# zyc00/Point-SAM

Hardware: AMD Instinct MI355X
Metric: point-clouds/sec (encode+1-prompt decode) (higher is better)
Workload: dtype f32 (fp32 in/out/accumulate; large GEMMs as row-scaled 2-way fp16 split x 3 MFMA products, fp32-grade error)

## Files before the change

### include/pointsam_hip.h

```cpp
#ifndef POINTSAM_HIP_H
#define POINTSAM_HIP_H

#include <stddef.h>
#include <stdint.h>

#ifdef __cplusplus
extern "C" {
#endif

typedef struct ihipStream_t* psam_stream_t;

#define PSAM_OK 0
#define PSAM_EINVAL (-1)
#define PSAM_EALIGN (-2)
#define PSAM_EWORKSPACE (-3)

#define PSAM_ACT_NONE 0
#define PSAM_ACT_GELU 1
#define PSAM_ACT_RELU 2
#define PSAM_ACT_SWIGLU 3

int32_t psam_version(void);
const char* psam_last_error_string(void);

// ... 62 lines not shown
#endif
#define PSAM_COUNTER_BYTES 65536
void psam_attention_f16x3_force_keysplit(int32_t mode);
int32_t psam_attention_f16x3_last_instance(void);
int32_t psam_attention_f16x3_last_keysplit(void);
int32_t psam_attention_f32_last_instance(void);
#ifdef PSAM_BUILD_EXPERIMENTS
void psam_twoway_decoder_force_fork(int32_t mode);
#endif
int32_t psam_gemm_f16x3p_fused_row_ln(int32_t N);
typedef struct {
    float* out_scale; float out_k1, out_k2; int32_t pack_out;
    float* stats; int32_t stat_cols;
    const float* ln_mean; const float* ln_rstd; const float* ln_c;
    float* gmax_out; int64_t gmax_ld; int32_t gmax_k; int32_t no_store;
    const float* row_ln_g; const float* row_ln_b; float row_ln_eps;
    const float* hyper; float* masks; int32_t hyper_c; int32_t hyper_rows;
    int64_t hyper_pstride;
    float* splitk_ws; int64_t splitk_plane; int32_t splitk;
    const float* out_bound;
    int32_t* counters;
} psam_gemm_fuse_t;
int32_t psam_gemm_f16x3p_splitk(int32_t M, int32_t N, int32_t K, int32_t act);
int32_t psam_gemm_f16x3p_hyper_planes(int32_t N, int32_t with_row_ln);
int32_t psam_sum_planes(const float* parts, int32_t P, int64_t pstride, int64_t count, float* out, psam_stream_t stream);
int32_t psam_gemm_f16x3p_stat_segs(int32_t N);
int32_t psam_gemm_f16x3p_ex(const void* A, int64_t lda, const float* scaleA, const void* W, int64_t ldw, const float* scaleW, float* C, int64_t ldc,
                            const float* bias, const float* residual, int64_t ldr, const float* rowbias, int64_t ldrb, int32_t rowgroup, int32_t M,
                            int32_t N, int32_t K, float alpha, int32_t act, const psam_gemm_fuse_t* fuse, psam_stream_t stream);
int32_t psam_ln_stats_finalize(const float* stats, int32_t rows, int32_t segs, int32_t cols, float eps, float* mean, float* rstd, psam_stream_t stream);
int32_t psam_linear128_ln_gelu_pack(const void* x, int64_t ldx, const float* x_scale, const void* w, int64_t ldw, const float* w_scale, const float* rowbias,
                                    int64_t ldrb, int32_t rowgroup, const float* gamma, const float* beta, float eps, float bound, int64_t rows, int32_t h1,
                                    void* out, int64_t ldo, float* out_scale, psam_stream_t stream);
int32_t psam_scale_pack_rows_g8(const float* X, int64_t ldx, int32_t rows, int32_t K, void* P, int64_t ldp, float* scale, psam_stream_t stream);
int32_t psam_linear(const float* x, int64_t ldx, const float* W, int64_t ldw, const float* bias, const float* residual, int64_t ldr, float* y,
                    int64_t ldy, int32_t M, int32_t N, int32_t K, int32_t act, psam_stream_t stream);
void psam_gemm_bf16x6_force_config(int32_t cfg);
void psam_gemm_force_config(int32_t cfg);

int32_t psam_layernorm(const float* x, int64_t ldx, const float* res, int64_t ldr, const float* w, const float* b, float* y, int64_t ldy,
                       int64_t rows, int32_t cols, float eps, int32_t act, psam_stream_t stream);
int32_t psam_layernorm_ex(const float* x, int64_t ldx, const float* res, int64_t ldr, const float* w, const float* b, float* y, int64_t ldy,
                          int64_t rows, int32_t cols, float eps, int32_t act, float* row_scale, int32_t pack, psam_stream_t stream);
int32_t psam_layernorm_ex2(const float* x, int64_t ldx, const float* res, int64_t ldr, const float* w, const float* b, float* y, int64_t ldy,
                           int64_t rows, int32_t cols, float eps, int32_t act, float* row_scale, int32_t pack, float* row_bound, float c2,
                           float c1, float c0, psam_stream_t stream);
int32_t psam_layernorm_rs(const float* x, int64_t ldx, const float* res, int64_t ldr, const float* w, const float* b, float* y, int64_t ldy,
                          int64_t rows, int32_t cols, float eps, int32_t act, float* row_scale, psam_stream_t stream);
int32_t psam_layernorm_last_instance(void);

int32_t psam_swiglu_ln(const float* gx, int64_t ldg, int32_t xoff, const float* w, const float* b, float* out, int64_t ldo, int64_t rows,
                       int32_t H, float eps, psam_stream_t stream);
int32_t psam_swiglu_ln_last_instance(void);

int32_t psam_attention_f32(const float* q, int64_t ldq, int64_t sq, const float* k, int64_t ldk, int64_t sk, const float* v, int64_t ldv,
                           int64_t sv, float* o, int64_t ldo, int64_t so, int32_t B, int32_t H, int32_t Lq, int32_t Lk, int32_t hd,
                           float scale, psam_stream_t stream);
int32_t psam_attention_f16x3(const float* q, int64_t ldq, int64_t sq, const float* k, int64_t ldk, int64_t sk, const float* v, int64_t ldv,
                           int64_t sv, float* o, int64_t ldo, int64_t so, int32_t B, int32_t H, int32_t Lq, int32_t Lk, int32_t hd,
                           float scale, psam_stream_t stream);
int32_t psam_attention_f16x3_ex(const float* q, int64_t ldq, int64_t sq, const float* k, int64_t ldk, int64_t sk, const float* v, int64_t ldv,
                                int64_t sv, float* o, int64_t ldo, int64_t so, int32_t B, int32_t H, int32_t Lq, int32_t Lk, int32_t hd, float scale,
                                const float* a_scale, float k1, float k2, float* o_scale, psam_stream_t stream);
size_t psam_attention_f16x3_keysplit_ws_bytes(int32_t B, int32_t H, int32_t Lq, int32_t Lk, int32_t hd, int32_t max_keysplit);
int32_t psam_attention_f16x3_ex2(const float* q, int64_t ldq, int64_t sq, const float* k, int64_t ldk, int64_t sk, const float* v, int64_t ldv,
                                int64_t sv, float* o, int64_t ldo, int64_t so, int32_t B, int32_t H, int32_t Lq, int32_t Lk, int32_t hd, float scale,
// ... 291 lines not shown
```

### point_sam_amd/_lib.py

```python
import ctypes
import os

_HERE = os.path.dirname(os.path.abspath(__file__))
LIB_PATH = os.environ.get("PSAM_HIP_LIB") or os.path.join(_HERE, "csrc", "libpointsam_hip.so")

i32, i64, f32 = ctypes.c_int32, ctypes.c_int64, ctypes.c_float
ptr, size_t = ctypes.c_void_p, ctypes.c_size_t

SIGNATURES = {
    "psam_version": (i32, []),
    "psam_last_error_string": (ctypes.c_char_p, []),
    "psam_fps_workspace_bytes": (size_t, [i32, i32, i32]),
    "psam_fps_set_cooperative": (None, [i32]),
    "psam_fps_set_pruning": (None, [i32]),
    "psam_fps": (i32, [ptr, i32, i32, i32, ptr, ptr, ptr, size_t, ptr]),
    "psam_knn": (i32, [ptr, ptr, i32, i32, i32, i32, ptr, ptr]),
    "psam_fps_last_instance": (i32, []),
    "psam_fps_last_grid_x": (i32, []),
    "psam_knn_force_band": (None, [i32]),
    "psam_knn_last_instance": (i32, []),
    "psam_three_nn": (i32, [ptr, ptr, i32, i32, i32, f32, ptr, ptr, ptr]),
    "psam_group_gather": (i32, [ptr, ptr, ptr, ptr, i32, i32, i32, i32, i32, i32, ptr, ptr]),
    "psam_group_gather_r": (i32, [ptr, ptr, ptr, ptr, i32, i32, i32, i32, i32, i32, f32, ptr, ptr]),
    "psam_group_gather_ld": (i32, [ptr, ptr, ptr, ptr, i32, i32, i32, i32, i32, i32, f32, ptr, i64, ptr]),
    "psam_patch_l1": (i32, [ptr, ptr, ptr, ptr, ptr, ptr, ptr, ptr, f32, i32, i32, i32, i32, i32, i32, ptr, ptr]),
    "psam_patch_l1_r": (i32, [ptr, ptr, ptr, ptr, ptr, ptr, ptr, ptr, f32, i32, i32, i32, i32, i32, i32, f32, ptr, ptr]),
    "psam_patch_l1_ex": (i32, [ptr, ptr, ptr, ptr, ptr, ptr, ptr, ptr, ptr, f32, i32, i32, i32, i32, i32, i32, f32, ptr, ptr, ptr]),
    "psam_error_regions": (i32, [ptr, ptr, ptr, ptr, i64, ptr]),
    "psam_border_farthest_workspace_bytes": (size_t, [i32, i32]),
    "psam_border_farthest": (i32, [ptr, ptr, i32, i32, i32, ptr, ptr, ptr, size_t, ptr]),
    "psam_group_max": (i32, [ptr, i64, ptr, i64, i64, i32, i32, ptr]),
    "psam_gemm_f32": (i32, [ptr, i64, i64, i64, ptr, i64, i64, i64, ptr, i64, i64, i64, ptr, ptr, i64, i64, i64, ptr, i64, i32,
                            i32, i32, i32, i32, i32, f32, i32, ptr]),
    "psam_gemm_bf16x6": (i32, [ptr, i64, i64, i64, ptr, i64, i64, i64, ptr, i64, i64, i64, ptr, ptr, i64, i64, i64, ptr, i64, i32,
                               i32, i32, i32, i32, i32, f32, i32, ptr]),
    "psam_linear": (i32, [ptr, i64, ptr, i64, ptr, ptr, i64, ptr, i64, i32, i32, i32, i32, ptr]),
    "psam_gemm_force_config": (None, [i32]),
    "psam_gemm_bf16x6_force_config": (None, [i32]),
    "psam_row_scale_f16": (i32, [ptr, i64, i32, i32, ptr, ptr]),
    "psam_pack_rows_f16x2_g8": (i32, [ptr, i64, ptr, i32, i32, ptr, i64, ptr]),
    "psam_gemm_f16x3p": (i32, [ptr, i64, ptr, ptr, i64, ptr, ptr, i64, ptr, ptr, i64, ptr, i64, i32, i32, i32, i32, f32, i32, ptr]),
    "psam_gemm_f16x3p_force_config": (None, [i32]),
    "psam_gemm_f16x3p_last_config": (i32, []),
    "psam_gemm_f16x3p_last_splitk": (i32, []),
    "psam_gemm_f16x3p_force_epilogue": (None, [i32]),
    "psam_gemm_f16x3p_force_splitk_fixup": (None, [i32]),
    "psam_gemm_f16x3p_force_continuous": (None, [i32]),
    "psam_attention_f16x3_force_keysplit": (None, [i32]),
    "psam_attention_f16x3_last_instance": (i32, []),
    "psam_attention_f16x3_last_keysplit": (i32, []),
    "psam_attention_f32_last_instance": (i32, []),
    "psam_twoway_decoder_force_fork": (None, [i32]),
    "psam_attention_packed_force_variant": (None, [i32]),
    "psam_attention_packed_force_nw": (None, [i32]),
    "psam_attention_packed_last_instance": (i32, []),
    "psam_gemm_f16x3p_fused_row_ln": (i32, [i32]),
    "psam_linear128_ln_gelu_pack": (i32, [ptr, i64, ptr, ptr, i64, ptr, ptr, i64, i32, ptr, ptr, f32, f32, i64, i32, ptr, i64, ptr, ptr]),
    "psam_gemm_f16x3p_stat_segs": (i32, [i32]),
    "psam_gemm_f16x3p_splitk": (i32, [i32, i32, i32, i32]),
    "psam_nn_group_feats": (i32, [ptr, ptr, ptr, ptr, ptr, i32, i32, i32, i32, i32, i32, ptr, i64, ptr]),
    "psam_scatter_amax": (i32, [ptr, i64, ptr, i64, i32, i64, i64, i32, ptr, i64, i32, ptr]),
    "psam_eva_block_prepared_bytes": (size_t, [i32, i32]),
    "psam_eva_block_prepare": (i32, [ptr, ptr, ptr, size_t, ptr]),
    "psam_eva_block_ws_bytes": (size_t, [i64, i32, i32]),
    "psam_eva_block": (i32, [ptr, ptr, ptr, i32, i32, ptr, size_t, ptr]),
    "psam_linear_skinny_multi": (i32, [ptr, i64, i64, i64, i32, i32, ptr]),
    "psam_linear_skinny_ln": (i32, [ptr, i64, ptr, i64, ptr, ptr, i64, ptr, ptr, f32, ptr, ptr, i64, i32, i32, i32, ptr, ptr]),
    "psam_linear_rows_multi": (i32, [ptr, i64, i64, i32, i32, i64, i64, i32, ptr]),
    "psam_linear_ln256": (i32, [ptr, i64, ptr, i64, ptr, ptr, i64, ptr, ptr, f32, ptr, i64, i64, i32, i32, ptr]),
    "psam_twoway_decoder_force_fast": (None, [i32]),
    "psam_scale_pack_rows_g8_add_dual": (i32, [ptr, i64, ptr, i64, i32, i32, i32, i32, ptr, ptr, ptr, ptr, i64, ptr]),
    "psam_mlp3_pair": (i32, [ptr, ptr, i32, ptr]),
    "psam_attention_small_force_split": (None, [i32]),
    "psam_attention_small_last_instance": (i32, []),
    "psam_layernorm_last_instance": (i32, []),
    "psam_swiglu_ln_last_instance": (i32, []),
    "psam_patch_l1_last_instance": (i32, []),
    "psam_interp3_last_instance": (i32, []),
    "psam_linear_skinny_ln_tmp_floats": (ctypes.c_size_t, [i32, i32]),
    "psam_scale_pack_rows_g8_add": (i32, [ptr, i64, ptr, i64, i32, i32, i32, i32, ptr, i64, ptr, ptr]),
    "psam_eva_gelu_block_prepared_bytes": (size_t, [i32, i32]),
    "psam_eva_gelu_block_prepare": (i32, [ptr, ptr, ptr, size_t, ptr]),
    "psam_eva_gelu_block_ws_bytes": (size_t, [i64, i32, i32]),
    "psam_eva_gelu_block": (i32, [ptr, ptr, ptr, i32, i32, ptr, size_t, ptr, ptr]),
    "psam_patch_encoder_prepared_bytes": (size_t, [i32, i32, i32]),
    "psam_patch_encoder_prepare": (i32, [ptr, ptr, ptr, size_t, ptr]),
    "psam_patch_encoder_ws_bytes": (size_t, [i64, i64, i32, i32]),
    "psam_patch_encoder": (i32, [ptr, ptr, ptr, ptr, ptr, ptr, ptr, i32, i32, i32, i32, i32, i32, f32, ptr, ptr, size_t, ptr]),
    "psam_upscale_masks_prepared_bytes": (size_t, [i32]),
    "psam_upscale_masks_prepare": (i32, [ptr, ptr, ptr, size_t, ptr]),
# ... 211 lines not shown
```

### point_sam_amd/build.py

```python
import os
import subprocess
import sys
from concurrent.futures import ThreadPoolExecutor

CSRC = os.path.join(os.path.dirname(os.path.abspath(__file__)), "csrc")
LIB = os.path.join(CSRC, "libpointsam_hip.so")
HIPCC = os.environ.get("HIPCC", "/opt/rocm/bin/hipcc")
ARCH = "gfx950"
COMMON = ["--offload-arch=" + ARCH, "-O3", "-std=c++17", "-fPIC", "-fvisibility=hidden", "-Wall", "-Wno-unused-function"]
EXPERIMENTS = os.environ.get("PSAM_BUILD_EXPERIMENTS", "0") == "1"
SOURCES = [
    ("tokenizer.hip", ["-ffp-contract=off"]),
    ("gemm.hip", []),
    ("gemm_split.hip", []),
    ("gemm_f16x3p.hip", []),
    ("gemm_f16x3pp.hip", []),
    ("patch_rowln.hip", []),
    ("attention.hip", []),
    ("rowops.hip", []),
    ("blocks.hip", []),
    ("masks.hip", []),
    ("scene.hip", ["-ffp-contract=off"]),
    ("regions.hip", ["-ffp-contract=off"]),
    ("crops.hip", ["-ffp-contract=off"]),
    ("scene_interp.hip", ["-ffp-contract=off"]),
    ("transfer.hip", ["-ffp-contract=off", "-fno-slp-vectorize"]),
    ("align.hip", ["-ffp-contract=off", "-fno-slp-vectorize"]),
    ("views.hip", ["-ffp-contract=off", "-fno-slp-vectorize"]),
    ("frames.hip", ["-ffp-contract=off", "-fno-slp-vectorize"]),
    ("fusion.hip", ["-ffp-contract=off", "-fno-slp-vectorize"]),
    ("geometry.hip", ["-ffp-contract=off", "-fno-slp-vectorize"]),
    ("error.cpp", ["-x", "hip"]),
] + ([("experiments/gemm_f16x3q.hip", ["-I" + CSRC]), ("experiments/gemm_f16x3s.hip", ["-I" + CSRC]), ("experiments/gemm_f16x3c.hip", ["-I" + CSRC]),
        ("experiments/twoway.hip", ["-I" + CSRC])] if EXPERIMENTS else [])
if EXPERIMENTS:
    COMMON = COMMON + ["-DPSAM_BUILD_EXPERIMENTS"]
FLAGS_STAMP = os.path.join(CSRC, ".build_flags")
PROBE_SRC = os.path.join(CSRC, "probe", "mfma_probe.hip")
PROBE_LIB = os.path.join(CSRC, "probe", "libpsam_probe.so")


def _stale(out, deps):
    return not os.path.exists(out) or any(os.path.getmtime(d) > os.path.getmtime(out) for d in deps)


def build_library(force: bool = False, verbose: bool = False) -> str:
    hdrs = [os.path.join(CSRC, f) for f in sorted(os.listdir(CSRC)) if f.endswith(".h")]
    hdrs.append(os.path.join(os.path.dirname(os.path.dirname(CSRC)), "include", "pointsam_hip.h"))
    flags = " ".join(COMMON)
    if (open(FLAGS_STAMP).read() != flags) if os.path.exists(FLAGS_STAMP) else EXPERIMENTS:
# ... 41 lines not shown
```

### point_sam_amd/csrc/blocks.hip

```cpp
#include <algorithm>
#include <cmath>
#include <cstring>
#include <initializer_list>
#ifdef PSAM_BUILD_EXPERIMENTS
#include <map>
#include <mutex>
#endif
#include <string>
#include <utility>
#include <vector>
#include "g8_pack.h"

namespace {
constexpr int64_t align256(int64_t b) { return (b + 255) / 256 * 256; }

struct Carve {
    char* base; int64_t off = 0;
    explicit Carve(void* p) : base(static_cast<char*>(p)) {}
    template <typename T> T* take(int64_t count) { T* r = base ? reinterpret_cast<T*>(base + off) : nullptr; off += align256(count * (int64_t)sizeof(T)); return r; }
    int64_t offset_of(const void* p) const { return static_cast<const char*>(p) - base; }
};
template <typename F> size_t carved_bytes(F&& layout) { Carve cv(nullptr); layout(cv); return (size_t)cv.off; }

struct Packed { float* w; float* s; };
// ... 401 lines not shown
    put_offsets(cv, p.c13, &plan->o_w13, &plan->o_s13); put_offsets(cv, p.c20m, &plan->o_w20m, &plan->o_s20m);
    put_offsets(cv, p.c20x, &plan->o_w20x, &plan->o_s20x); put_offsets(cv, p.c23, &plan->o_w23, &plan->o_s23);
    int32_t rc = pack_weight(WHO, wt->c13_w, h0, h0, h0, p.c13, stream);
    if (!rc) rc = pack_weight(WHO, wt->c20_w, 2 * h0, h1, h0, p.c20m, stream);
    if (!rc) rc = pack_weight(WHO, wt->c20_w + h0, 2 * h0, h1, h0, p.c20x, stream);
    if (!rc) rc = pack_weight(WHO, wt->c23_w, h1, cout, h1, p.c23, stream);
    return packing_done(WHO, rc, stream);
#undef WHO
}

PSAM_API size_t psam_patch_encoder_ws_bytes(int64_t rows, int64_t groups, int32_t h0, int32_t h1) {
    if (rows <= 0 || groups <= 0 || h0 <= 0 || h1 <= 0) return 0;
    return carved_bytes([&](Carve& cv) { patch_ws(cv, rows, groups, h0, h1); });
}

PSAM_API int32_t psam_patch_encoder(const psam_patch_encoder_plan_t* plan, const void* prepared, const float* xyz, const float* feats, const float* centers,
                                    const int64_t* knn_idx, const int64_t* center_idx, int32_t B, int32_t rep, int32_t N, int32_t G, int32_t K, int32_t C,
                                    float radius, float* out, void* ws, size_t ws_bytes, hipStream_t stream) {
    PSAM_REQUIRE(plan && prepared && xyz && feats && centers && knn_idx && out && ws, PSAM_EINVAL, "psam_patch_encoder: null pointer");
    const int h0 = plan->h0, h1 = plan->h1, cout = plan->cout, a = kpad32(h0), b = kpad32(h1);
    const int64_t groups = (int64_t)B * rep * G, rows = groups * K;
    PSAM_REQUIRE(B > 0 && rep > 0 && N > 0 && G > 0 && (K == 32 || (K > 0 && K % 64 == 0)) && rows % 256 == 0 && rows < ((int64_t)1 << 31), PSAM_EINVAL,
                 "psam_patch_encoder: group size must be 32 or a multiple of 64, and B * rep * G * K a multiple of 256");
    const int Kp = K <= 64 ? K : 64, parts = K / Kp;
    PSAM_REQUIRE(plan->cin == 3 + C * (center_idx ? 2 : 1), PSAM_EINVAL, "psam_patch_encoder: feature channels do not match the first Linear");
    PSAM_REQUIRE(ws_bytes >= psam_patch_encoder_ws_bytes(rows, groups, h0, h1), PSAM_EWORKSPACE, "psam_patch_encoder: workspace too small");
    auto P = [&](int64_t off) { return at(prepared, off); };
    Carve cv(ws);
    const PatchWs w = patch_ws(cv, rows, groups, h0, h1);
    float* part1 = parts > 1 ? w.x3 : w.y1;
    float* part2 = parts > 1 ? w.x1 : out;
    PSAM_REQUIRE(parts == 1 || ((int64_t)groups * parts * h0 <= rows * b && (int64_t)groups * parts * cout <= rows * a), PSAM_EINVAL,
                 "psam_patch_encoder: partial maxima do not fit the workspace");
    int32_t rc = psam_patch_l1_ex(xyz, feats, centers, knn_idx, center_idx, plan->c10_w, plan->c10_b, plan->c11_w, plan->c11_b, plan->eps, B, rep, N, G, K, C, radius, w.x1, w.s1, stream);
    if (rc) return rc;
    psam_gemm_fuse_t f;
    std::memset(&f, 0, sizeof(f));
    f.pack_out = 1; f.out_scale = w.s2; f.out_k1 = plan->k1; f.out_k2 = plan->k2; f.gmax_out = part1; f.gmax_ld = h0; f.gmax_k = Kp;
    rc = psam_gemm_f16x3p_ex(w.x1, a, w.s1, P(plan->o_w13), a, P(plan->o_s13), w.x2, a, plan->c13_b, nullptr, 0, nullptr, 0, 0, (int32_t)rows, h0, a, 1.f, 0, &f, stream);
    if (rc) return rc;
    if (parts > 1) { rc = psam_group_max(part1, h0, w.y1, h0, groups, parts, h0, stream); if (rc) return rc; }
    const Lin c20m{plan->c20_w, 2 * h0, plan->c20_b, P(plan->o_w20m), P(plan->o_s20m), h1, h0};
    rc = host_linear(c20m, w.y1, groups, w.g1, 0, G, w.y1p, w.sy, stream);
    if (rc) return rc;
    if (h1 == 512 && rows % 128 == 0 && psam_gemm_f16x3p_fused_row_ln(h1)) {
        std::memset(&f, 0, sizeof(f));
        f.row_ln_g = plan->c21_w; f.row_ln_b = plan->c21_b; f.row_ln_eps = plan->eps; f.pack_out = 1; f.out_scale = w.rs; f.out_k1 = 0.f; f.out_k2 = plan->ln21_bound;
        rc = psam_gemm_f16x3p_ex(w.x2, a, w.s2, P(plan->o_w20x), a, P(plan->o_s20x), w.x3, b, nullptr, nullptr, 0, w.g1, h1, K, (int32_t)rows, h1, a, 1.f, PSAM_ACT_GELU, &f, stream);
        if (rc) return rc;
    } else if (h0 == 128 && h1 == 512 && rows % 64 == 0) {
        rc = psam_linear128_ln_gelu_pack(w.x2, a, w.s2, P(plan->o_w20x), a, P(plan->o_s20x), w.g1, h1, K, plan->c21_w, plan->c21_b, plan->eps, plan->ln21_bound, rows, h1,
                                         w.x3, b, w.rs, stream);
        if (rc) return rc;
    } else {
        rc = psam_gemm_f16x3p_ex(w.x2, a, w.s2, P(plan->o_w20x), a, P(plan->o_s20x), w.x3, h1, nullptr, nullptr, 0, w.g1, h1, K, (int32_t)rows, h1, a, 1.f, 0, nullptr, stream);
        if (rc) return rc;
        rc = psam_layernorm_ex(w.x3, h1, nullptr, 0, plan->c21_w, plan->c21_b, w.x3, b, rows, h1, plan->eps, PSAM_ACT_GELU, w.rs, 1, stream);
        if (rc) return rc;
    }
    std::memset(&f, 0, sizeof(f));
    f.gmax_out = part2; f.gmax_ld = cout; f.gmax_k = Kp; f.no_store = 1;
    rc = psam_gemm_f16x3p_ex(w.x3, b, w.rs, P(plan->o_w23), b, P(plan->o_s23), out, cout, plan->c23_b, nullptr, 0, nullptr, 0, 0, (int32_t)rows, cout, b, 1.f, 0, &f, stream);
    if (rc || parts == 1) return rc;
    return psam_group_max(part2, cout, out, cout, groups, parts, cout, stream);
}

namespace {
struct UpscalePrepared { Packed u0, u3; };
UpscalePrepared upscale_prepared(Carve& cv, int dim) { return {take_packed(cv, dim, dim), take_packed(cv, dim, dim)}; }

struct UpscaleWs { float *kp, *k1, *sk, *up, *s1, *parts; };
UpscaleWs upscale_ws(Carve& cv, int64_t Z, int N, int G, int C, int dim) {
    const int64_t a = kpad32(dim), planes = psam_gemm_f16x3p_hyper_planes(dim, 0);
// ... 416 lines not shown
```

### point_sam_amd/csrc/g8_pack.h

```cpp
#pragma once
#include "common.h"

typedef unsigned u32x4 __attribute__((ext_vector_type(4)));

static inline __host__ __device__ int kpad32(int k) { return (k + 31) & ~31; }

#ifdef __HIPCC__
typedef float psam_f32x2 __attribute__((ext_vector_type(2)));
typedef float psam_f32x4 __attribute__((ext_vector_type(4)));
typedef _Float16 psam_f16x2 __attribute__((ext_vector_type(2)));

__device__ __forceinline__ void g8_split2_scaled(const psam_f32x2 xs, unsigned& hi, unsigned& lo) {
    const psam_f16x2 h = __builtin_convertvector(xs, psam_f16x2);
    const psam_f32x2 r = xs - __builtin_convertvector(h, psam_f32x2);
    hi = __builtin_bit_cast(unsigned, h);
    lo = __builtin_bit_cast(unsigned, __builtin_convertvector(r, psam_f16x2));
}
__device__ __forceinline__ void psam_split2_f16(float x0, float x1, float s, unsigned& hi, unsigned& lo) { g8_split2_scaled(psam_f32x2{x0, x1} * s, hi, lo); }

__device__ __forceinline__ float g8_absmax4(const psam_f32x4 v) { return fmaxf(fmaxf(fabsf(v[0]), fabsf(v[1])), fmaxf(fabsf(v[2]), fabsf(v[3]))); }
__device__ __forceinline__ float g8_absmax4(float amax, const psam_f32x4 v) { return fmaxf(fmaxf(amax, fmaxf(fabsf(v[0]), fabsf(v[1]))), fmaxf(fabsf(v[2]), fabsf(v[3]))); }
__device__ __forceinline__ float g8_row_scale(float lane_max) { return f16_row_scale(wave_max(lane_max)); }

template <int DIST, bool SHFL = false>
// ... 26 lines not shown
    g8_split2_scaled(xs23, h1, l1);
    return g8_chunk_words<DIST>(h0, l0, h1, l1, lane);
}

struct g8_group { u32x4 hi, lo; };
__device__ __forceinline__ g8_group g8_halfwave_group(const psam_f32x4 x, const psam_f32x4 y, float s) {
    unsigned xh[2], xl[2], yh[2], yl[2];
    psam_split2_f16(x[0], x[1], s, xh[0], xl[0]);
    psam_split2_f16(x[2], x[3], s, xh[1], xl[1]);
    psam_split2_f16(y[0], y[1], s, yh[0], yl[0]);
    psam_split2_f16(y[2], y[3], s, yh[1], yl[1]);
    psam_swap32(xh[0], yh[0]); psam_swap32(xh[1], yh[1]); psam_swap32(xl[0], yl[0]); psam_swap32(xl[1], yl[1]);
    return {u32x4{xh[0], xh[1], yh[0], yh[1]}, u32x4{xl[0], xl[1], yl[0], yl[1]}};
}
__device__ __forceinline__ g8_group g8_whole_group(const float (&v)[8], float s) {
    unsigned hi[4], lo[4];
#pragma unroll
    for (int e = 0; e < 4; ++e) psam_split2_f16(v[2 * e], v[2 * e + 1], s, hi[e], lo[e]);
    return {u32x4{hi[0], hi[1], hi[2], hi[3]}, u32x4{lo[0], lo[1], lo[2], lo[3]}};
}
__device__ __forceinline__ void g8_store_group(unsigned* first, const g8_group& g) {
    *reinterpret_cast<u32x4*>(first) = g.hi;
    *reinterpret_cast<u32x4*>(first + 4) = g.lo;
}
__device__ __forceinline__ void g8_store_halfwave_group(unsigned* first, const psam_f32x4 x, const psam_f32x4 y, float s) { g8_store_group(first, g8_halfwave_group(x, y, s)); }

__device__ __forceinline__ void g8_store_pair(unsigned* P, int64_t row, int ld, int lane, float x0, float x1, float s) {
    unsigned hi, lo;
    psam_split2_f16(x0, x1, s, hi, lo);
    unsigned* o = P + row * ld + (lane >> 2) * 8 + (lane & 3);
    o[0] = hi;
    o[4] = lo;
}
#endif
```

### point_sam_amd/model.py

```python
import math
from dataclasses import dataclass, field
from types import SimpleNamespace
from typing import Optional

import torch

from . import ops
from .config import ModelConfig
from .ops import ACT_GELU, ACT_NONE, ACT_RELU
from .streams import pipeline_streams
from .weights import check_state_dict


def _round_up(x, m):
    return (x + m - 1) // m * m


@dataclass
class TokenizerState:
    fps_idx: torch.Tensor
    centers: torch.Tensor
    knn_idx: torch.Tensor
    interp_index: torch.Tensor
    interp_weight: torch.Tensor
# ... 162 lines not shown
            if cfg.vit.swiglu and ops.EvaBlock.supported(D, cfg.vit.heads, cfg.vit.mlp_hidden):
                for blk in self.blocks:
                    blk.c_block = ops.EvaBlock(w, blk.p, D, cfg.vit.heads, cfg.vit.mlp_hidden, cfg.vit.ln_eps)
            elif not cfg.vit.swiglu and ops.EvaGeluBlock.supported(D, cfg.vit.heads, cfg.vit.mlp_hidden):
                for blk in self.blocks:
                    blk.c_block = ops.EvaGeluBlock(w, blk.p, D, cfg.vit.heads, cfg.vit.mlp_hidden, cfg.vit.ln_eps)
            torch.cuda.current_stream(self.device).synchronize()

    def _lin(self, name, x, **kw):
        return ops.linear(x, self.fw.get(name + ".weight", self.w[name + ".weight"]), self.w.get(name + ".bias"), **kw)

    def _ln(self, name, x, eps, **kw):
        return ops.layernorm(x, self.w[name + ".weight"], self.w[name + ".bias"], eps, **kw)

    def _ln_feeds_gemm(self, x, consumer):
        if self.precision != "f16x3" or x.shape[0] < ops.SPLIT_MIN_M or (consumer + ".weight") not in self.fw or not ops.layernorm_can_pack(x.shape[1]) \
                or x.shape[1] % 32 != 0:
            return False, None
        return True, torch.empty(x.shape[0], dtype=torch.float32, device=x.device)

    def _patch_encoder(self, prefix, coords, feats, centers, knn_idx, radius=None, center_idx=None):
        w, eps = self.w, self.cfg.ln_eps
        K = knn_idx.shape[2]
        h0 = self.cfg.patch_hidden[0]
        rows = feats.shape[0] * knn_idx.shape[1] * K
        l1 = (w[prefix + ".conv1.0.weight"], w[prefix + ".conv1.0.bias"], w[prefix + ".conv1.1.weight"], w[prefix + ".conv1.1.bias"], eps)
        w2a = w[prefix + ".conv2.0.weight"]
        fused = (self.precision == "f16x3" and self.fuse_patch and (K in (32, 64) or K % 64 == 0) and ops.fuse_supported(rows, 128) and prefix in self.pe_bound
                 and all((prefix + n) in self.fw for n in (".conv1.3.weight", ".conv2.0.weight#x", ".conv2.3.weight")))
        if fused and self.c_blocks and prefix in getattr(self, "c_patch", {}) and ops.current_gemm_mode() == "f16x3":
            return self.c_patch[prefix].run(coords, feats, centers, knn_idx, radius=radius, center_idx=center_idx)
        if fused:
            groups = rows // K
            s1 = torch.empty(rows, dtype=torch.float32, device=coords.device)
            h1 = ops.patch_l1(coords, feats, centers, knn_idx, *l1, radius=radius, center_idx=center_idx, scale_out=s1)
            h2 = torch.empty(rows, h0, dtype=torch.float32, device=coords.device)
            s2 = torch.empty(rows, dtype=torch.float32, device=coords.device)
            Kp = K if K <= 64 else 64
            parts = K // Kp
            y1 = torch.empty(groups * parts, h0, dtype=torch.float32, device=coords.device)
            k1, k2 = self.pe_bound[prefix]
            self._lin(prefix + ".conv1.3", h1, x_scale=s1, x_packed=True, out=h2, pack_out=(s2, k1, k2), group_max_out=y1, group_max_k=Kp)
            if parts > 1:
                y1 = ops.group_max(y1, parts)
            del h1
            g1 = ops.linear(y1, self.fw.get(prefix + ".conv2.0.weight#max", w2a[:, :h0]), w[prefix + ".conv2.0.bias"])
            hd1 = w2a.shape[0]
            if ops.fused_row_ln(hd1) and hd1 == 512 and (prefix + ".conv2.3.weight") in self.fw and rows % 128 == 0:
                h3 = torch.empty(rows, hd1, dtype=torch.float32, device=coords.device)
                rs, pk = torch.empty(rows, dtype=torch.float32, device=coords.device), True
                bound = self.ln_bound.get(prefix)
                if bound is None:
                    bound = self.ln_bound.setdefault(prefix, 1.001 * ops.row_ln_bound(w[prefix + ".conv2.1.weight"], w[prefix + ".conv2.1.bias"]) + 1e-30)
                ops.linear(h2, self.fw[prefix + ".conv2.0.weight#x"], None, act=ACT_GELU, rowbias=g1, rowgroup=K, x_scale=s2, x_packed=True, out=h3,
                           row_ln=(w[prefix + ".conv2.1.weight"], w[prefix + ".conv2.1.bias"], eps), pack_out=(rs, 0.0, bound))
                del h2
            elif ops.linear128_ln_gelu_supported(rows, h0, hd1, K) and (prefix + ".conv2.3.weight") in self.fw and ops.current_gemm_mode() == "f16x3":
                h3 = torch.empty(rows, hd1, dtype=torch.float32, device=coords.device)
                rs, pk = torch.empty(rows, dtype=torch.float32, device=coords.device), True
                bound = self.ln_bound.get(prefix)
                if bound is None:
                    bound = self.ln_bound.setdefault(prefix, 1.001 * ops.row_ln_bound(w[prefix + ".conv2.1.weight"], w[prefix + ".conv2.1.bias"]) + 1e-30)
                ops.linear128_ln_gelu_pack(h2, s2, self.fw[prefix + ".conv2.0.weight#x"], g1, K, w[prefix + ".conv2.1.weight"], w[prefix + ".conv2.1.bias"], eps, bound,
                                           h3, rs)
                del h2
            else:
                h3 = ops.linear(h2, self.fw[prefix + ".conv2.0.weight#x"], None, rowbias=g1, rowgroup=K, x_scale=s2, x_packed=True)
                del h2
                pk, rs = self._ln_feeds_gemm(h3, prefix + ".conv2.3")
                self._ln(prefix + ".conv2.1", h3, eps, act=ACT_GELU, out=h3, scale_out=rs, pack=pk)
            emb = torch.empty(groups * parts, self.w[prefix + ".conv2.3.weight"].shape[0], dtype=torch.float32, device=coords.device)
            self._lin(prefix + ".conv2.3", h3, x_scale=rs, x_packed=pk, group_max_out=emb, group_max_k=Kp, no_store=True)
            return ops.group_max(emb, parts) if parts > 1 else emb
        h1 = ops.patch_l1(coords, feats, centers, knn_idx, *l1, radius=radius, center_idx=center_idx)
        h2 = self._lin(prefix + ".conv1.3", h1)
        del h1
        y1 = ops.group_max(h2, K)
        g1 = ops.linear(y1, self.fw.get(prefix + ".conv2.0.weight#max", w2a[:, :h0]), w[prefix + ".conv2.0.bias"])
# ... 539 lines not shown
```

### point_sam_amd/ops.py

```python
import ctypes
import torch

from . import _lib
from ._lib import check

ACT_NONE, ACT_GELU, ACT_RELU, ACT_SWIGLU = 0, 1, 2, 3

GEMM_PROFILE = None
GEMM_PROFILE_EVERY = 29
GEMM_PROFILE_OTHERS = ()
GEMM_PROFILE_AFTER = 0
_gemm_counter = 0


def _sample_now():
    return GEMM_PROFILE is not None and _gemm_counter > GEMM_PROFILE_AFTER and _gemm_counter % GEMM_PROFILE_EVERY == 0


def _sampled_launch(launch, record):
    cur = torch.cuda.current_stream()
    for o in GEMM_PROFILE_OTHERS:
        cur.wait_stream(o)
    s, e = torch.cuda.Event(enable_timing=True), torch.cuda.Event(enable_timing=True)
    s.record()
# ... 168 lines not shown
    check(_lib.load().psam_three_nn(xyz.data_ptr(), centers.data_ptr(), B, N, G, eps, idx.data_ptr(), w.data_ptr(), _stream()), "psam_three_nn")
    return idx, w


def group_gather(xyz, feats, centers, knn_idx, radius=None, width=None):
    _chk(xyz); _chk(feats); _chk(centers); _chk(knn_idx, torch.int64)
    B, N, _ = xyz.shape
    rep = feats.shape[0] // B
    G, K = knn_idx.shape[1:]
    C = feats.shape[-1]
    width = width or 3 + C
    out = torch.empty(B * rep, G, K, width, dtype=torch.float32, device=xyz.device)
    check(_lib.load().psam_group_gather_ld(xyz.data_ptr(), feats.data_ptr(), centers.data_ptr(), knn_idx.data_ptr(), B, rep, N, G, K, C,
                                           float(radius or 0.0), out.data_ptr(), width, _stream()), "psam_group_gather")
    return out


def patch_l1(xyz, feats, centers, knn_idx, W, bias, lnw, lnb, eps, out=None, radius=None, center_idx=None, scale_out=None):
    _chk(xyz); _chk(feats); _chk(centers); _chk(knn_idx, torch.int64); _chk(W)
    B, N, _ = xyz.shape
    rep = feats.shape[0] // B
    G, K = knn_idx.shape[1:]
    C = feats.shape[-1]
    cin = 3 + C * (2 if center_idx is not None else 1)
    assert W.shape == (128, cin), (W.shape, cin)
    if center_idx is not None:
        _chk(center_idx, torch.int64, "center_idx")
    rows = B * rep * G * K
    if out is None:
        out = torch.empty(rows, 128, dtype=torch.float32, device=xyz.device)
    check(_lib.load().psam_patch_l1_ex(xyz.data_ptr(), feats.data_ptr(), centers.data_ptr(), knn_idx.data_ptr(), _p(center_idx), W.data_ptr(),
                                       bias.data_ptr(), lnw.data_ptr(), lnb.data_ptr(), eps, B, rep, N, G, K, C, float(radius or 0.0), out.data_ptr(),
                                       _p(scale_out), _stream()), "psam_patch_l1")
    return out


def nn_group_feats(xyz, centers, nn_idx, feats=None, logits=None, width=8):
    _chk(xyz); _chk(centers); _chk(nn_idx, torch.int64)
    B, N, _ = xyz.shape
    G = centers.shape[1]
    if logits is None:
        _chk(feats)
        C, rep, mode = feats.shape[-1], 1, 0
    else:
        _chk(logits)
        C, rep, mode = 0, logits.shape[0] // B, 1
    assert width % 4 == 0 and width >= (4 + C if mode == 0 else 5)
    out = torch.empty(B * rep * N, width, dtype=torch.float32, device=xyz.device)
    check(_lib.load().psam_nn_group_feats(xyz.data_ptr(), centers.data_ptr(), nn_idx.data_ptr(), _p(feats), _p(logits), B, rep, N, G, C, mode, out.data_ptr(),
                                          width, _stream()), "psam_nn_group_feats")
    return out


def scatter_amax(x, idx, out_rows, rows_per_set, set_stride, idx_rep=1, include_self=False):
    xp, ldx = _row_view(x, "x"); _chk(idx, torch.int64)
    R, C = x.shape
    out = torch.empty(out_rows, C, dtype=torch.float32, device=x.device)
    check(_lib.load().psam_scatter_amax(xp, ldx, idx.data_ptr(), R, C, rows_per_set, set_stride, idx_rep, out.data_ptr(), out_rows, int(bool(include_self)),
                                        _stream()), "psam_scatter_amax")
    return out


def group_max(x: torch.Tensor, K: int, out=None):
    _chk(x)
    rows, C = x.shape
    groups = rows // K
# ... 1665 lines not shown
```

Measured before the change: 811.2.

## Fuse patch L1 layer, LayerNorm+GELU and conv1.3 GEMM into one persistent kernel

Adds a persistent patch_front kernel. Each block gathers neighbour points and features, computes the small first linear layer, applies LayerNorm and GELU, and packs the result into fp16 hi/lo splits in shared memory. It then runs the 128x128 conv1.3 GEMM with MFMA, writing packed output, row scales and per-group maxima. This removes the intermediate h1 round trip through global memory and one kernel launch, and it prefetches the next block's gather indices and raw inputs. The kernel only handles h0=128 with C of 1 or 3, and it gives up the tuned generic GEMM path, so occupancy and register pressure may suffer.

```diff
diff --git a/include/pointsam_hip.h b/include/pointsam_hip.h
--- a/include/pointsam_hip.h
+++ b/include/pointsam_hip.h
@@ -118,6 +118,10 @@
 int32_t psam_linear128_ln_gelu_pack(const void* x, int64_t ldx, const float* x_scale, const void* w, int64_t ldw, const float* w_scale, const float* rowbias,
                                     int64_t ldrb, int32_t rowgroup, const float* gamma, const float* beta, float eps, float bound, int64_t rows, int32_t h1,
                                     void* out, int64_t ldo, float* out_scale, psam_stream_t stream);
+int32_t psam_patch_front(const float* xyz, const float* feats, const float* centers, const int64_t* knn_idx, const int64_t* center_idx, const float* W,
+                         const float* bias, const float* lnw, const float* lnb, float eps, const void* w13, int64_t ldw, const float* w13_scale, const float* b13,
+                         float k1, float k2, int32_t B, int32_t rep, int32_t N, int32_t G, int32_t K, int32_t C, float radius, int32_t h0, void* out, int64_t ldo,
+                         float* out_scale, float* gmax_out, int64_t gmax_ld, psam_stream_t stream);
 int32_t psam_scale_pack_rows_g8(const float* X, int64_t ldx, int32_t rows, int32_t K, void* P, int64_t ldp, float* scale, psam_stream_t stream);
 int32_t psam_linear(const float* x, int64_t ldx, const float* W, int64_t ldw, const float* bias, const float* residual, int64_t ldr, float* y,
                     int64_t ldy, int32_t M, int32_t N, int32_t K, int32_t act, psam_stream_t stream);
diff --git a/point_sam_amd/_lib.py b/point_sam_amd/_lib.py
--- a/point_sam_amd/_lib.py
+++ b/point_sam_amd/_lib.py
@@ -56,6 +56,8 @@
     "psam_attention_packed_last_instance": (i32, []),
     "psam_gemm_f16x3p_fused_row_ln": (i32, [i32]),
     "psam_linear128_ln_gelu_pack": (i32, [ptr, i64, ptr, ptr, i64, ptr, ptr, i64, i32, ptr, ptr, f32, f32, i64, i32, ptr, i64, ptr, ptr]),
+    "psam_patch_front": (i32, [ptr, ptr, ptr, ptr, ptr, ptr, ptr, ptr, ptr, f32, ptr, i64, ptr, ptr, f32, f32, i32, i32, i32, i32, i32, i32, f32, i32, ptr, i64, ptr,
+                               ptr, i64, ptr]),
     "psam_gemm_f16x3p_stat_segs": (i32, [i32]),
     "psam_gemm_f16x3p_splitk": (i32, [i32, i32, i32, i32]),
     "psam_nn_group_feats": (i32, [ptr, ptr, ptr, ptr, ptr, i32, i32, i32, i32, i32, i32, ptr, i64, ptr]),
diff --git a/point_sam_amd/build.py b/point_sam_amd/build.py
--- a/point_sam_amd/build.py
+++ b/point_sam_amd/build.py
@@ -16,6 +16,7 @@
     ("gemm_f16x3p.hip", []),
     ("gemm_f16x3pp.hip", []),
     ("patch_rowln.hip", []),
+    ("patch_front.hip", ["-ffp-contract=off"]),
     ("attention.hip", []),
     ("rowops.hip", []),
     ("blocks.hip", []),
diff --git a/point_sam_amd/csrc/blocks.hip b/point_sam_amd/csrc/blocks.hip
--- a/point_sam_amd/csrc/blocks.hip
+++ b/point_sam_amd/csrc/blocks.hip
@@ -457,13 +457,20 @@
     float* part2 = parts > 1 ? w.x1 : out;
     PSAM_REQUIRE(parts == 1 || ((int64_t)groups * parts * h0 <= rows * b && (int64_t)groups * parts * cout <= rows * a), PSAM_EINVAL,
                  "psam_patch_encoder: partial maxima do not fit the workspace");
-    int32_t rc = psam_patch_l1_ex(xyz, feats, centers, knn_idx, center_idx, plan->c10_w, plan->c10_b, plan->c11_w, plan->c11_b, plan->eps, B, rep, N, G, K, C, radius, w.x1, w.s1, stream);
-    if (rc) return rc;
+    int32_t rc;
     psam_gemm_fuse_t f;
-    std::memset(&f, 0, sizeof(f));
-    f.pack_out = 1; f.out_scale = w.s2; f.out_k1 = plan->k1; f.out_k2 = plan->k2; f.gmax_out = part1; f.gmax_ld = h0; f.gmax_k = Kp;
-    rc = psam_gemm_f16x3p_ex(w.x1, a, w.s1, P(plan->o_w13), a, P(plan->o_s13), w.x2, a, plan->c13_b, nullptr, 0, nullptr, 0, 0, (int32_t)rows, h0, a, 1.f, 0, &f, stream);
-    if (rc) return rc;
+    if (h0 == 128 && rows % 64 == 0 && (C == 1 || C == 3)) {
+        rc = psam_patch_front(xyz, feats, centers, knn_idx, center_idx, plan->c10_w, plan->c10_b, plan->c11_w, plan->c11_b, plan->eps, P(plan->o_w13), a,
+                              (const float*)P(plan->o_s13), plan->c13_b, plan->k1, plan->k2, B, rep, N, G, K, C, radius, h0, w.x2, a, w.s2, part1, h0, stream);
+        if (rc) return rc;
+    } else {
+        rc = psam_patch_l1_ex(xyz, feats, centers, knn_idx, center_idx, plan->c10_w, plan->c10_b, plan->c11_w, plan->c11_b, plan->eps, B, rep, N, G, K, C, radius, w.x1, w.s1, stream);
+        if (rc) return rc;
+        std::memset(&f, 0, sizeof(f));
+        f.pack_out = 1; f.out_scale = w.s2; f.out_k1 = plan->k1; f.out_k2 = plan->k2; f.gmax_out = part1; f.gmax_ld = h0; f.gmax_k = Kp;
+        rc = psam_gemm_f16x3p_ex(w.x1, a, w.s1, P(plan->o_w13), a, P(plan->o_s13), w.x2, a, plan->c13_b, nullptr, 0, nullptr, 0, 0, (int32_t)rows, h0, a, 1.f, 0, &f, stream);
+        if (rc) return rc;
+    }
     if (parts > 1) { rc = psam_group_max(part1, h0, w.y1, h0, groups, parts, h0, stream); if (rc) return rc; }
     const Lin c20m{plan->c20_w, 2 * h0, plan->c20_b, P(plan->o_w20m), P(plan->o_s20m), h1, h0};
     rc = host_linear(c20m, w.y1, groups, w.g1, 0, G, w.y1p, w.sy, stream);
diff --git a/point_sam_amd/csrc/g8_pack.h b/point_sam_amd/csrc/g8_pack.h
--- a/point_sam_amd/csrc/g8_pack.h
+++ b/point_sam_amd/csrc/g8_pack.h
@@ -82,4 +82,13 @@
     o[0] = hi;
     o[4] = lo;
 }
+__device__ __forceinline__ void g8_pair_words(float x0, float x1, float s, unsigned& hi, unsigned& lo) { psam_split2_f16(x0, x1, s, hi, lo); }
+__device__ __forceinline__ unsigned g8_column_word(float xs, int lane) {
+    const _Float16 h = (_Float16)xs;
+    const _Float16 l = (_Float16)(xs - (float)h);
+    const unsigned hb = __builtin_bit_cast(unsigned short, h), lb = __builtin_bit_cast(unsigned short, l);
+    const bool upper = lane & 1;
+    const unsigned got = (unsigned)dpp_i32<DPP_XOR1>((int)(upper ? hb : lb));
+    return upper ? (got | (lb << 16)) : (hb | (got << 16));
+}
 #endif
diff --git a/point_sam_amd/csrc/patch_front.hip b/point_sam_amd/csrc/patch_front.hip
--- /dev/null
+++ b/point_sam_amd/csrc/patch_front.hip
@@ -0,0 +1,244 @@
+#include "g8_pack.h"
+#include "gemm_f16x3p_args.h"
+#include "gemm_epilogue_t.h"
+
+namespace {
+struct FrontArgs {
+    const float* xyz; const float* feats; const float* centers; const int64_t* knn_idx; const int64_t* center_idx;
+    const float* W10; const float* b10; const float* lnw; const float* lnb;
+    const unsigned char* W13; const float* sw13; const float* b13;
+    unsigned* out; float* out_scale; float* gmax;
+    int64_t ldw, ldo, ldg;
+    int rep, N, G, K, gmax_k, nblocks;
+    float eps, inv_radius, k1, k2;
+};
+
+constexpr int PF_ROWS = 64, PF_H = 128, PF_WAVES = 8;
+constexpr int PF_ROWB = 128;
+constexpr int PF_SLAB = PF_ROWS * PF_ROWB;
+constexpr int PF_STAGE = (PF_H / 32) * PF_SLAB;
+constexpr int PF_INW = 12;
+
+__device__ __forceinline__ void pf_barrier() { asm volatile("s_waitcnt lgkmcnt(0)\n\ts_barrier" ::: "memory"); }
+
+template <int CIN, bool CENTRAL>
+__global__ __launch_bounds__(64 * PF_WAVES, 4) void patch_front_kernel(const FrontArgs p) {
+#pragma clang fp contract(off)
+    constexpr int C = CENTRAL ? (CIN - 3) / 2 : CIN - 3;
+    constexpr int NRAW = 6 + (CENTRAL ? 2 * C : C);
+    __shared__ __attribute__((aligned(16))) unsigned char stage[PF_STAGE];
+    __shared__ __attribute__((aligned(16))) float inl[2 * PF_ROWS * PF_INW];
+    __shared__ __attribute__((aligned(16))) float w10l[(CIN + 1) * PF_H];
+    __shared__ __attribute__((aligned(16))) float rsql[PF_ROWS], sol[PF_ROWS];
+    __shared__ float pmax[PF_H];
+    const int tid = threadIdx.x, lane = tid & 63;
+    const int wave = __builtin_amdgcn_readfirstlane(tid >> 6);
+    const int ti = wave & 1, tj = wave >> 1;
+
+    auto row_of = [&](int blk, unsigned& gi, unsigned& k) {
+        const unsigned row = (unsigned)blk * PF_ROWS + wave * 8 + (lane & 7);
+        gi = row / (unsigned)p.K; k = row - gi * (unsigned)p.K;
+    };
+    auto load_index = [&](int blk) {
+        unsigned gi, k;
+        row_of(blk, gi, k);
+        const unsigned g = gi % (unsigned)p.G, b = (gi / (unsigned)p.G) / (unsigned)p.rep;
+        return (int)p.knn_idx[((int64_t)b * p.G + g) * p.K + k];
+    };
+    auto load_raw = [&](int blk, int n, float (&raw)[NRAW]) {
+        unsigned gi, k;
+        row_of(blk, gi, k);
+        const unsigned g = gi % (unsigned)p.G, bf = gi / (unsigned)p.G, b = bf / (unsigned)p.rep;
+        const float* pt = p.xyz + ((int64_t)b * p.N + n) * 3;
+        const float* c = p.centers + ((int64_t)b * p.G + g) * 3;
+        const float* f = p.feats + ((int64_t)bf * p.N + n) * C;
+#pragma unroll
+        for (int i = 0; i < 3; ++i) { raw[i] = pt[i]; raw[3 + i] = c[i]; }
+#pragma unroll
+        for (int i = 0; i < C; ++i) raw[6 + i] = f[i];
+        if constexpr (CENTRAL) {
+            const float* fc = p.feats + ((int64_t)bf * p.N + p.center_idx[(int64_t)b * p.G + g]) * C;
+#pragma unroll
+            for (int i = 0; i < C; ++i) raw[6 + C + i] = fc[i];
+        }
+    };
+    auto put_inputs = [&](const float (&raw)[NRAW], int st) {
+        if (lane < 8) {
+            float* o = inl + (st * PF_ROWS + wave * 8 + lane) * PF_INW;
+#pragma unroll
+            for (int i = 0; i < 3; ++i) o[i] = (raw[i] - raw[3 + i]) * p.inv_radius;
+#pragma unroll
+            for (int i = 0; i < C; ++i) o[3 + i] = raw[6 + i];
+            if constexpr (CENTRAL) {
+#pragma unroll
+                for (int i = 0; i < C; ++i) o[3 + C + i] = raw[6 + i] - raw[6 + C + i];
+            }
+        }
+    };
+
+    int blk = blockIdx.x;
+    const int step = gridDim.x;
+    int nidx;
+    {
+        float raw[NRAW];
+        load_raw(blk, load_index(blk), raw);
+        nidx = blk + step < p.nblocks ? load_index(blk + step) : 0;
+        put_inputs(raw, 0);
+    }
+    if (tid < PF_H) {
+#pragma unroll
+        for (int i = 0; i < CIN; ++i) w10l[i * PF_H + tid] = p.W10[tid * CIN + i];
+        w10l[CIN * PF_H + tid] = p.b10[tid];
+    }
+    const float g0 = p.lnw[2 * lane], g1 = p.lnw[2 * lane + 1], e0 = p.lnb[2 * lane], e1 = p.lnb[2 * lane + 1];
+
+    pf16x8 fw[8][2];
+    {
+        const unsigned char* wl = p.W13 + (int64_t)(tj * 32 + (lane & 31)) * p.ldw * 4 + (lane >> 5) * 32;
+#pragma unroll
+        for (int ks = 0; ks < 8; ++ks)
+#pragma unroll
+            for (int q = 0; q < 2; ++q) fw[ks][q] = *reinterpret_cast<const pf16x8*>(wl + ks * 64 + q * 16);
+    }
+    const float isw = inv_pow2(p.sw13[tj * 32 + (lane & 31)]), b13 = p.b13[tj * 32 + (lane & 31)];
+
+    pf_barrier();
+    for (int st = 0; blk < p.nblocks; blk += step, st ^= 1) {
+        const bool has_next = blk + step < p.nblocks;
+        const int64_t row0 = (int64_t)blk * PF_ROWS;
+        float raw[NRAW];
+        load_raw(has_next ? blk + step : blk, nidx, raw);
+        nidx = blk + 2 * step < p.nblocks ? load_index(blk + 2 * step) : 0;
+
+        constexpr int R = 2;
+#pragma unroll 1
+        for (int rr = 0; rr < 8 / R; ++rr) {
+            int lf = lane;
+            asm volatile("" : "+v"(lf));
+            const float* wl = w10l + 2 * lf;
+            float y0[R], y1[R];
+            {
+                const psam_f32x2 bb = *reinterpret_cast<const psam_f32x2*>(wl + CIN * PF_H);
+                const float* in = inl + (st * PF_ROWS + wave * 8 + rr * R) * PF_INW;
+#pragma unroll
+                for (int q = 0; q < R; ++q) { y0[q] = bb[0]; y1[q] = bb[1]; }
+#pragma unroll
+                for (int i = 0; i < CIN; ++i) {
+                    if (CIN > 6 && i % 3 == 0 && i > 0) ept_fence();
+                    const psam_f32x2 w = *reinterpret_cast<const psam_f32x2*>(wl + i * PF_H);
+#pragma unroll
+                    for (int q = 0; q < R; ++q) { y0[q] = fmaf(w[0], in[q * PF_INW + i], y0[q]); y1[q] = fmaf(w[1], in[q * PF_INW + i], y1[q]); }
+                }
+            }
+            float mean[R], var[R];
+#pragma unroll
+            for (int q = 0; q < R; ++q) mean[q] = wave_sum(y0[q] + y1[q]) * (1.0f / 128.0f);
+#pragma unroll
+            for (int q = 0; q < R; ++q) { y0[q] -= mean[q]; y1[q] -= mean[q]; var[q] = wave_sum(y0[q] * y0[q] + y1[q] * y1[q]) * (1.0f / 128.0f); }
+            float o0[R], o1[R], sc[R];
+#pragma unroll
+            for (int q = 0; q < R; ++q) {
+                const float r = 1.0f / sqrtf(var[q] + p.eps);
+                o0[q] = gelu_erf(y0[q] * r * g0 + e0); o1[q] = gelu_erf(y1[q] * r * g1 + e1);
+            }
+#pragma unroll
+            for (int q = 0; q < R; ++q) sc[q] = f16_row_scale(wave_max(fmaxf(fabsf(o0[q]), fabsf(o1[q]))));
+#pragma unroll
+            for (int q = 0; q < R; ++q) {
+                const int r = wave * 8 + rr * R + q;
+                unsigned hi, lo;
+                g8_pair_words(o0[q], o1[q], sc[q], hi, lo);
+                unsigned char* sb = stage + (lf >> 4) * PF_SLAB + r * PF_ROWB + ((lf & 3) << 2);
+                const int ch = 2 * ((lf >> 2) & 3), swz = (r >> 1) & 7;
+                *reinterpret_cast<unsigned*>(sb + ((ch ^ swz) << 4)) = hi;
+                *reinterpret_cast<unsigned*>(sb + (((ch + 1) ^ swz) << 4)) = lo;
+                if (lane == 0) {
+                    const float rs = inv_pow2(sc[q]), so = f16_row_scale(p.k1 * rs + p.k2);
+                    rsql[r] = rs; sol[r] = so;
+                    p.out_scale[row0 + r] = so;
+                }
+            }
+        }
+        put_inputs(raw, st ^ 1);
+        pf_barrier();
+
+        pf32x16 acc;
+#pragma unroll
+        for (int r = 0; r < 16; ++r) acc[r] = 0.f;
+        int lm = lane;
+        asm volatile("" : "+v"(lm));
+        {
+            const unsigned char* sa = stage + ti * 32 * PF_ROWB + (lm & 31) * PF_ROWB;
+            const int swz = (lm >> 1) & 7, hq = 2 * (lm >> 5);
+            auto frag = [&](int ks, int q) { return *reinterpret_cast<const pf16x8*>(sa + (ks >> 1) * PF_SLAB + (((4 * (ks & 1) + hq + q) ^ swz) << 4)); };
+            pf16x8 fa[2] = {frag(0, 0), frag(0, 1)};
+#pragma unroll
+            for (int ks = 0; ks < 8; ++ks) {
+                pf16x8 fn[2] = {fa[0], fa[1]};
+                if (ks < 7) { fn[0] = frag(ks + 1, 0); fn[1] = frag(ks + 1, 1); }
+                constexpr int PA[3] = {0, 1, 0}, PW[3] = {1, 0, 0};
+#pragma unroll
+                for (int t = 0; t < 3; ++t) acc = __builtin_amdgcn_mfma_f32_32x32x16_f16(fa[PA[t]], fw[ks][PW[t]], acc, 0, 0, 0);
+                ept_fence();
+                fa[0] = fn[0]; fa[1] = fn[1];
+            }
+        }
+        const int c = lm & 31, h = lm >> 5;
+        const bool upper = c & 1;
+        float gm = -INFINITY;
+        unsigned* ob = p.out + (row0 + ti * 32 + 4 * h) * p.ldo + tj * 32 + 8 * (c >> 3) + (upper ? 4 : 0) + ((c & 7) >> 1);
+#pragma unroll
+        for (int g = 0; g < 4; ++g) {
+            ept_fence();
+            const ep_f32x4 rq = ep_load4(rsql + ti * 32 + 8 * g + 4 * h), sv = ep_load4(sol + ti * 32 + 8 * g + 4 * h);
+#pragma unroll
+            for (int e = 0; e < 4; ++e) {
+                const float v = __builtin_fmaf(acc[4 * g + e] * rq[e], isw, b13);
+                gm = fmaxf(gm, v);
+                ob[(int64_t)e * p.ldo] = g8_column_word(v * sv[e], lm);
+            }
+            ob += 8 * p.ldo;
+        }
+        {
+            float a = gm, b = gm;
+            ept_swap32f(a, b);
+            gm = fmaxf(a, b);
+        }
+        if (p.gmax_k == 32) {
+            if (h == 0) p.gmax[(row0 / 32 + ti) * p.ldg + tj * 32 + c] = gm;
+        } else if (ti == 1 && h == 0) {
+            pmax[tj * 32 + c] = gm;
+        }
+        pf_barrier();
+        if (p.gmax_k != 32 && ti == 0 && h == 0) p.gmax[(row0 / 64) * p.ldg + tj * 32 + c] = fmaxf(gm, pmax[tj * 32 + c]);
+    }
+}
+}
+
+PSAM_API int32_t psam_patch_front(const float* xyz, const float* feats, const float* centers, const int64_t* knn_idx, const int64_t* center_idx, const float* W,
+                                  const float* bias, const float* lnw, const float* lnb, float eps, const void* w13, int64_t ldw, const float* w13_scale,
+                                  const float* b13, float k1, float k2, int32_t B, int32_t rep, int32_t N, int32_t G, int32_t K, int32_t C, float radius, int32_t h0,
+                                  void* out, int64_t ldo, float* out_scale, float* gmax_out, int64_t gmax_ld, hipStream_t stream) {
+#define WHO "psam_patch_front"
+    PSAM_REQUIRE(xyz && feats && centers && knn_idx && W && bias && lnw && lnb && w13 && w13_scale && b13 && out && out_scale && gmax_out, PSAM_EINVAL,
+                 WHO ": null pointer");
+    PSAM_REQUIRE(h0 == PF_H, PSAM_EINVAL, WHO ": hidden_dims[0] must be 128");
+    PSAM_REQUIRE(C == 1 || C == 3, PSAM_EINVAL, WHO ": C must be 1 (mask logit) or 3 (rgb)");
+    PSAM_REQUIRE(B > 0 && rep > 0 && N > 0 && G > 0 && (K == 32 || (K > 0 && K % 64 == 0)), PSAM_EINVAL, WHO ": bad shape (group size 32 or a multiple of 64)");
+    const int64_t rows = (int64_t)B * rep * G * K;
+    PSAM_REQUIRE(rows % PF_ROWS == 0 && rows < ((int64_t)1 << 31), PSAM_EINVAL, WHO ": B * rep * G * K must be a multiple of 64 below 2^31");
+    PSAM_REQUIRE(ldw >= PF_H && ldo >= PF_H && gmax_ld >= PF_H, PSAM_EINVAL, WHO ": rows of 128 columns expected (ldw, ldo, gmax_ld >= 128)");
+    PSAM_REQUIRE(((ldw | ldo) & 7) == 0 && (((uintptr_t)w13 | (uintptr_t)out) & 31) == 0, PSAM_EALIGN, WHO ": packed rows must be 32-byte aligned");
+    FrontArgs p;
+    p.xyz = xyz; p.feats = feats; p.centers = centers; p.knn_idx = knn_idx; p.center_idx = center_idx; p.W10 = W; p.b10 = bias; p.lnw = lnw; p.lnb = lnb;
+    p.W13 = (const unsigned char*)w13; p.sw13 = w13_scale; p.b13 = b13; p.out = (unsigned*)out; p.out_scale = out_scale; p.gmax = gmax_out;
+    p.ldw = ldw; p.ldo = ldo; p.ldg = gmax_ld; p.rep = rep; p.N = N; p.G = G; p.K = K; p.gmax_k = K == 32 ? 32 : 64; p.nblocks = (int)(rows / PF_ROWS);
+    p.eps = eps; p.inv_radius = radius > 0.f ? 1.0f / radius : 1.0f; p.k1 = k1; p.k2 = k2;
+    const int grid = p.nblocks < 2 * psam_cu_count() ? p.nblocks : 2 * psam_cu_count();
+#define PF_LAUNCH(CIN, CEN) hipLaunchKernelGGL((patch_front_kernel<CIN, CEN>), dim3((unsigned)grid), dim3(64 * PF_WAVES), 0, stream, p)
+    if (center_idx) { if (C == 3) PF_LAUNCH(9, true); else PF_LAUNCH(5, true); }
+    else { if (C == 3) PF_LAUNCH(6, false); else PF_LAUNCH(4, false); }
+#undef PF_LAUNCH
+    return psam_launch_status(WHO ": launch failed");
+#undef WHO
+}
diff --git a/point_sam_amd/model.py b/point_sam_amd/model.py
--- a/point_sam_amd/model.py
+++ b/point_sam_amd/model.py
@@ -218,18 +218,22 @@
             return self.c_patch[prefix].run(coords, feats, centers, knn_idx, radius=radius, center_idx=center_idx)
         if fused:
             groups = rows // K
-            s1 = torch.empty(rows, dtype=torch.float32, device=coords.device)
-            h1 = ops.patch_l1(coords, feats, centers, knn_idx, *l1, radius=radius, center_idx=center_idx, scale_out=s1)
             h2 = torch.empty(rows, h0, dtype=torch.float32, device=coords.device)
             s2 = torch.empty(rows, dtype=torch.float32, device=coords.device)
             Kp = K if K <= 64 else 64
             parts = K // Kp
             y1 = torch.empty(groups * parts, h0, dtype=torch.float32, device=coords.device)
             k1, k2 = self.pe_bound[prefix]
-            self._lin(prefix + ".conv1.3", h1, x_scale=s1, x_packed=True, out=h2, pack_out=(s2, k1, k2), group_max_out=y1, group_max_k=Kp)
+            if ops.patch_front_supported(rows, h0, K, feats.shape[-1]) and ops.current_gemm_mode() == "f16x3":
+                ops.patch_front(coords, feats, centers, knn_idx, *l1, self.fw[prefix + ".conv1.3.weight"], w[prefix + ".conv1.3.bias"], k1, k2, h2, s2, y1,
+                                radius=radius, center_idx=center_idx)
+            else:
+                s1 = torch.empty(rows, dtype=torch.float32, device=coords.device)
+                h1 = ops.patch_l1(coords, feats, centers, knn_idx, *l1, radius=radius, center_idx=center_idx, scale_out=s1)
+                self._lin(prefix + ".conv1.3", h1, x_scale=s1, x_packed=True, out=h2, pack_out=(s2, k1, k2), group_max_out=y1, group_max_k=Kp)
+                del h1
             if parts > 1:
                 y1 = ops.group_max(y1, parts)
-            del h1
             g1 = ops.linear(y1, self.fw.get(prefix + ".conv2.0.weight#max", w2a[:, :h0]), w[prefix + ".conv2.0.bias"])
             hd1 = w2a.shape[0]
             if ops.fused_row_ln(hd1) and hd1 == 512 and (prefix + ".conv2.3.weight") in self.fw and rows % 128 == 0:
diff --git a/point_sam_amd/ops.py b/point_sam_amd/ops.py
--- a/point_sam_amd/ops.py
+++ b/point_sam_amd/ops.py
@@ -224,6 +224,31 @@
     check(_lib.load().psam_patch_l1_ex(xyz.data_ptr(), feats.data_ptr(), centers.data_ptr(), knn_idx.data_ptr(), _p(center_idx), W.data_ptr(),
                                        bias.data_ptr(), lnw.data_ptr(), lnb.data_ptr(), eps, B, rep, N, G, K, C, float(radius or 0.0), out.data_ptr(),
                                        _p(scale_out), _stream()), "psam_patch_l1")
+    return out
+
+
+def patch_front_supported(rows: int, h0: int, K: int, C: int) -> bool:
+    return h0 == 128 and rows > 0 and rows % 64 == 0 and C in (1, 3) and (K == 32 or (K > 0 and K % 64 == 0))
+
+
+def patch_front(xyz, feats, centers, knn_idx, W, bias, lnw, lnb, eps, fw13, b13, k1, k2, out, scale_out, group_max_out, radius=None, center_idx=None):
+    _chk(xyz); _chk(feats); _chk(centers); _chk(knn_idx, torch.int64); _chk(W)
+    B, N, _ = xyz.shape
+    rep = feats.shape[0] // B
+    G, K = knn_idx.shape[1:]
+    C = feats.shape[-1]
+    cin = 3 + C * (2 if center_idx is not None else 1)
+    assert W.shape == (128, cin), (W.shape, cin)
+    if center_idx is not None:
+        _chk(center_idx, torch.int64, "center_idx")
+    rows = B * rep * G * K
+    op, ldo = _row_view(out, "out")
+    gp, ldg = _row_view(group_max_out, "group_max_out")
+    assert out.shape[0] == rows and scale_out.numel() == rows and group_max_out.shape[0] * min(K, 64) == rows, (out.shape, scale_out.shape, group_max_out.shape)
+    check(_lib.load().psam_patch_front(xyz.data_ptr(), feats.data_ptr(), centers.data_ptr(), knn_idx.data_ptr(), _p(center_idx), W.data_ptr(), bias.data_ptr(),
+                                       lnw.data_ptr(), lnb.data_ptr(), eps, fw13.packed.data_ptr(), fw13.packed.stride(0), fw13.scale.data_ptr(), b13.data_ptr(),
+                                       float(k1), float(k2), B, rep, N, G, K, C, float(radius or 0.0), fw13.N, op, ldo, scale_out.data_ptr(), gp, ldg, _stream()),
+          "psam_patch_front")
     return out
 
 
```

New measurement: 813.5 (median of 6 runs). Within noise of the previous version (+0.3%).
